# robjermy/CMVS-PMVS

Hardware: AMD Instinct MI355X
Metric: refined patches/sec + NCC evals/sec, 50-view 4K synthetic, 1/2/4/8 GPU (higher is better)
Workload: dtype f32 (f64 optimizer)

## Files before the change

cmvs-pmvs_amd/csrc/pmvs_api.cpp:

```cpp
#include <hip/hip_runtime.h>

#include <algorithm>
#include <climits>
#include <cmath>
#include <cstdarg>
#include <cstdio>
#include <cstdlib>
#include <cstring>
#include <chrono>
#include <condition_variable>
#include <mutex>
#include <string>
#include <vector>

#include "../../include/pmvs_amd.h"
#include "pmvs_features.h"
#include "pmvs_fmt.h"
#include "pmvs_launch.h"

using namespace pmvsdev;

namespace {

thread_local std::string g_err = "";
// ... 1615 lines not shown
  HIPCHK(hipSetDevice(sc->device));
  ExportTemp tmp;
  pmvs_patch* dP = nullptr;
  if (n) {
    EXPCHK(tmp.alloc(&dP, (size_t)n));
    EXPCHK(hipMemcpyAsync(dP, patches, (size_t)n * sizeof(pmvs_patch), hipMemcpyHostToDevice, sc->stream));
  }
  return text_records(sc, dP, n, sz, kind, flags, index2image, out, cap, bytes);
}

pmvs_status pmvs_selftest_format(int32_t device, int32_t precision, const float* in, int32_t n, char* out, int32_t* len) {
  if (!in || !out || !len || n <= 0 || (precision != 6 && precision != 17)) return fail(PMVS_EINVAL, "invalid argument");
  if (device == -1) {
    std::memset(out, 0, (size_t)n * 24);
    for (int i = 0; i < n; ++i) len[i] = pmvsfmt::fmt_g(in[i], precision, out + (size_t)i * 24);
    return PMVS_OK;
  }
  HIPCHK(hipSetDevice(device));
  ExportTemp tmp;
  float* d_in = nullptr;
  char* d_out = nullptr;
  int* d_len = nullptr;
  EXPCHK(tmp.alloc(&d_in, (size_t)n));
  EXPCHK(tmp.alloc(&d_out, (size_t)n * 24));
  EXPCHK(tmp.alloc(&d_len, (size_t)n));
  EXPCHK(hipMemcpy(d_in, in, (size_t)n * sizeof(float), hipMemcpyHostToDevice));
  EXPCHK(hipMemset(d_out, 0, (size_t)n * 24));
  EXPCHK(launch_format_selftest(precision, d_in, n, d_out, d_len, nullptr));
  EXPCHK(hipMemcpy(out, d_out, (size_t)n * 24, hipMemcpyDeviceToHost));
  EXPCHK(hipMemcpy(len, d_len, (size_t)n * sizeof(int), hipMemcpyDeviceToHost));
  return PMVS_OK;
}

pmvs_status pmvs_scene_set_shard(pmvs_scene* sc, int32_t rank, int32_t world, pmvs_allgather_fn fn, void* ctx) {
  if (!sc || world < 1 || rank < 0 || rank >= world || (world > 1 && !fn)) return fail(PMVS_EINVAL, "invalid shard");
  sc->shard_rank = rank;
  sc->shard_world = world;
  sc->shard_fn = fn;
  sc->shard_ctx = ctx;
  sc->shard_rccl = nullptr;
  return PMVS_OK;
}

pmvs_status pmvs_scene_set_cluster(pmvs_scene* sc, int32_t rank, int32_t world, const int32_t* image_ids,
                                   pmvs_allgather_fn fn, void* ctx) {
  if (!sc || world < 1 || rank < 0 || rank >= world || (world > 1 && (!fn || !image_ids)))
    return fail(PMVS_EINVAL, "invalid cluster");
  sc->cl_world = 1;
  sc->cl_fn = nullptr;
  sc->cl_rccl = nullptr;
  if (world == 1) return PMVS_OK;
  const int num = sc->ds.num, tnum = sc->ds.tnum;
  pmvs_status bad = PMVS_OK;
  int maxid = -1;
  std::vector<int> id2idx;
  if (tnum > PMVS_MAX_TARGETS) bad = fail(PMVS_EUNSUPPORTED, "cluster: more than %d target images", PMVS_MAX_TARGETS);
  for (int i = 0; i < num && !bad; ++i) {
    if (image_ids[i] < 0) bad = fail(PMVS_EINVAL, "image_ids[%d] = %d", i, image_ids[i]);
    maxid = std::max(maxid, image_ids[i]);
  }
  if (!bad && maxid > (1 << 26)) bad = fail(PMVS_EUNSUPPORTED, "image number %d", maxid);
  if (!bad) {
    id2idx.assign((size_t)maxid + 1, -1);
    for (int i = 0; i < num && !bad; ++i) {
      if (id2idx[image_ids[i]] >= 0) bad = fail(PMVS_EINVAL, "image number %d appears twice", image_ids[i]);
      id2idx[image_ids[i]] = i;
// ... 105 lines not shown
```

cmvs-pmvs_amd/csrc/pmvs_filter.hip:

```cpp
#include <hip/hip_runtime.h>
#include <hipcub/hipcub.hpp>

#include <algorithm>
#include <chrono>
#include <cmath>
#include <cstdio>
#include <cstddef>
#include <cstdlib>
#include <cstring>
#include <functional>
#include <mutex>
#include <unordered_map>
#include <vector>

#include "pmvs_device.h"
#include "pmvs_launch.h"
#include "pmvs_layout.h"
#include "pmvs_queue.h"

namespace pmvsdev {

#ifndef PMVS_NB_CAP
#define PMVS_NB_CAP 1024
#endif
// ... 2515 lines not shown
  FCHK(memset_big(B.cellcnt, 0, (c.ncells + 1) * sizeof(int), c.st));
  if (e > 0) {
    hipLaunchKernelGGL(cell_hist_kernel, dim3(nblk(e)), dim3(256), 0, c.st, B.keys2, e, B.cellcnt);
    hipLaunchKernelGGL(items_kernel, dim3(nblk(e)), dim3(256), 0, c.st, B.keys2, e, items);
  }
  FCHK(cub_run(B.temp, [&](void* t, size_t& tb) {
    return hipcub::DeviceScan::ExclusiveSum(t, tb, B.cellcnt.p, csr_off, (int)(c.ncells + 1), c.st);
  }));
  return hipGetLastError();
}

__global__ void flag_order_kernel(const int* __restrict__ v, const int* __restrict__ order, int na, int* __restrict__ f) {
  const int i = blockIdx.x * blockDim.x + threadIdx.x;
  if (i < na) f[i] = v[order[i]] != 0;
}
__global__ void scatter_order_kernel(const int* __restrict__ f, const int* __restrict__ off, const int* __restrict__ order,
                                     int na, int* __restrict__ out) {
  const int i = blockIdx.x * blockDim.x + threadIdx.x;
  if (i < na && f[i]) out[off[i]] = order[i];
}

__global__ void pack_bits_kernel(const int* __restrict__ f, int n, unsigned* __restrict__ bits) {
  const int w = blockIdx.x * blockDim.x + threadIdx.x;
  if (w * 32 >= n) return;
  unsigned v = 0u;
  for (int b = 0; b < 32 && w * 32 + b < n; ++b) v |= (f[w * 32 + b] != 0 ? 1u : 0u) << b;
  bits[w] = v;
}
__global__ void unpack_bits_kernel(const unsigned* __restrict__ bits, int n, int* __restrict__ f) {
  const int k = blockIdx.x * blockDim.x + threadIdx.x;
  if (k < n) f[k] = (bits[k >> 5] >> (k & 31)) & 1u;
}

static int lab_jump() {
  static const int v = getenv("PMVS_LAB_JUMP") ? std::max(1, atoi(getenv("PMVS_LAB_JUMP"))) : 1;
  return v;
}
__global__ void lab_init_kernel(int* __restrict__ lab, int* __restrict__ active, int na) {
  const int i = blockIdx.x * blockDim.x + threadIdx.x;
  if (i < na) {
    lab[i] = i;
    active[i] = 1;
  }
}
__global__ void lab_relax_kernel(const int* __restrict__ eoff, const int* __restrict__ edges, int na, int* lab,
                                 int* active, int all, int* changed, int jump) {
  const int i = blockIdx.x * blockDim.x + threadIdx.x;
  if (i >= na) return;
  if (!all && !jump && active[i] == 0) return;
  const int l0 = lab[i], l1 = lab[l0];
  const bool jumped = l1 < l0 && atomicMin(&lab[i], l1) > l1;
  if (jumped) atomicOr(changed, 1);
  if (!all && !jumped && active[i] == 0) return;
  if (atomicExch(&active[i], 0) == 0 && !all && !jumped) return;
  const int li = atomicAdd(&lab[i], 0);
  bool any = false;
  for (int e = eoff[i]; e < eoff[i + 1]; ++e) {
    const int j = edges[e];
    if (li < lab[j] && atomicMin(&lab[j], li) > li) {
      atomicOr(&active[j], 1);
      any = true;
    }
  }
  if (any) atomicOr(changed, 1);
}
__global__ void lab_count_kernel(const int* __restrict__ lab, int na, int* __restrict__ csize) {
  const int i = blockIdx.x * blockDim.x + threadIdx.x;
  const int l = (i < na) ? lab[i] : -1;
  const int l0 = __shfl(l, 0, 64);
  const unsigned long long same = __ballot(i < na && l == l0);
  if (i < na && l != l0) atomicAdd(&csize[l], 1);
  if ((threadIdx.x & 63) == 0 && same) atomicAdd(&csize[l0], (int)__popcll(same));
}
__global__ void lab_flags_kernel(const int* __restrict__ lab, const int* __restrict__ csize, const int* __restrict__ order,
                                 int na, int threshold, int* __restrict__ flags) {
  const int i = blockIdx.x * blockDim.x + threadIdx.x;
  if (i < na && csize[lab[i]] < threshold) flags[order[i]] = 1;
}

static hipError_t collect(Ctx& c) {
  FilterBuffers& B = c.B;
  FCHK(hipMemsetAsync(B.counters, 0, 8 * sizeof(int), c.st));
  hipLaunchKernelGGL(first_cell_kernel, dim3(std::min(nblk((long long)c.n * kLG), 2048u)), dim3(256), 0, c.st, c.s, c.P, c.n,
                     B.preg, B.tgoff, B.keys,
                     B.counters);
  FCHK(cub_run(B.temp, [&](void* t, size_t& tb) {
    return hipcub::DeviceRadixSort::SortKeys(t, tb, B.keys.p, B.keys2.p, c.n, 32, 32 + cell_bits(c.ncells), c.st);
  }));
  FCHK(read_int(B.counters, &c.nalive, c.st));
  FCHK(hipMemsetAsync(B.rank, 0xff, c.n * sizeof(int), c.st));
  if (c.nalive > 0)
    hipLaunchKernelGGL(rank_kernel, dim3(nblk(c.nalive)), dim3(256), 0, c.st, B.keys2, c.nalive, B.order, B.rank);
  hipLaunchKernelGGL(hot_kernel, dim3(nblk(c.n)), dim3(256), 0, c.st, c.s, c.P, c.n, B.hot);
  return hipGetLastError();
}

static hipError_t set_dm_vgrids(Ctx& c, int additive) {
// ... 230 lines not shown
    }
    fprintf(stderr, "[filter] neighbours: max unique %d, overflowed %d of %d; first: %d %d %d\n", mx, ov, c.nalive,
            cnts[ord[0]], c.nalive > 1 ? cnts[ord[1]] : 0, c.nalive > 2 ? cnts[ord[2]] : 0);
  }
  FCHK(read_int(B.counters + 3, overflow, st));
  if (part) {
    long long ovf = 0;
    FCHK(merge_flags(*overflow, &ovf));
    *overflow = (int)ovf;
    if (inject && inj_where == 'g') return hipErrorOutOfMemory;
  }
  {
    int errs[2] = {0, 0};
    FCHK(hipMemcpy(errs, B.counters + 6, 2 * sizeof(int), hipMemcpyDeviceToHost));
    if (errs[0]) {
      fprintf(stderr, "[filter] neighbor kernel bounds violations: %d (first code %d)\n", errs[0], errs[1]);
      return hipErrorIllegalAddress;
    }
  }
  FCHK(apply_flags(c, &counts[2]));
  FCHK(set_dm_vgrids(c, 1));
  if (c.nalive) {
    const int na = c.nalive;
    hipLaunchKernelGGL(group_edges_kernel, dim3(nblk(na)), dim3(256), 0, st, s, c.dev(), 0, B.edge_off, B.cnt, B.edges);
    FCHK(hipMemsetAsync(B.cnt + na, 0, sizeof(int), st));
    FCHK(cub_run(B.temp, [&](void* t, size_t& tb) { return hipcub::DeviceScan::ExclusiveSum(t, tb, B.cnt.p, B.edge_off.p, na + 1, st); }));
    int ne = 0;
    FCHK(read_int(B.edge_off + na, &ne, st));
    if ((size_t)ne > B.edges.cap) FCHK(B.edges.alloc((size_t)ne * 2));
    hipLaunchKernelGGL(group_edges_kernel, dim3(nblk(na)), dim3(256), 0, st, s, c.dev(), 1, B.edge_off, B.cnt, B.edges);
    const int threshold = std::max(20, na / 10000);
    int* lab = B.need;
    int* csize = B.list;
    int* changed = B.counters + 5;
    int* active = B.list;
    hipLaunchKernelGGL(lab_init_kernel, dim3(nblk(na)), dim3(256), 0, st, lab, active, na);
    int sweep = 0;
    for (int it = 0;; ++it) {
      const bool verify = (it % 9) == 8;
      FCHK(hipMemsetAsync(changed, 0, sizeof(int), st));
      for (int r = 0; r < (verify ? 1 : 8); ++r) {
        if (ne)
          hipLaunchKernelGGL(lab_relax_kernel, dim3(nblk(na)), dim3(256), 0, st, B.edge_off, B.edges, na, lab, active,
                             verify ? 1 : 0, changed, (sweep++ % lab_jump()) == 0 ? 1 : 0);
      }
      int ch = 0;
      FCHK(read_int(changed, &ch, st));
      if (verify && !ch) break;
      if (!verify && !ch) it = 9 * (it / 9) + 7;
      if (it > 9 * (na + 1)) return hipErrorIllegalState;
    }
    FCHK(hipMemsetAsync(csize, 0, na * sizeof(int), st));
    hipLaunchKernelGGL(lab_count_kernel, dim3(nblk(na)), dim3(256), 0, st, lab, na, csize);
    FCHK(hipMemsetAsync(B.flags, 0, n * sizeof(int), st));
    hipLaunchKernelGGL(lab_flags_kernel, dim3(nblk(na)), dim3(256), 0, st, lab, csize, B.order, na, threshold, B.flags);
    hipLaunchKernelGGL(flag_rank_kernel, dim3(nblk(na)), dim3(256), 0, st, dP, B.order, na);
    hipLaunchKernelGGL(clear_fixed_kernel, dim3(nblk(n)), dim3(256), 0, st, dP, n, B.flags);
    FCHK(apply_flags(c, &counts[3]));
  }
  dbg(st, "groups");
  FCHK(set_dm_vgrids(c, 1));
  FCHK(build_lists(c, 0));
  FCHK(collect(c));
  hipLaunchKernelGGL(keep_kernel, dim3(nblk(n)), dim3(256), 0, st, n, B.preg, B.rank, keep_dev);
  int lovf = 0;
  FCHK(read_int(B.counters + 8, &lovf, st));
  if (lovf) return hipErrorNotSupported;
  return hipGetLastError();
}

static void nb_prof_dump(const char* what) {
#if defined(NB_PROFILE)
  unsigned long long h[3][8];
  if (hipDeviceSynchronize() != hipSuccess || hipMemcpyFromSymbol(h, HIP_SYMBOL(g_nb_prof), sizeof(h)) != hipSuccess) return;
  fprintf(stderr, "{\"nb_prof\": \"%s\"", what);
  for (int k = 0; k < 3; ++k) {
    fprintf(stderr, ", \"k%d\": [", k);
    for (int i = 0; i < 8; ++i) fprintf(stderr, "%s%llu", i ? ", " : "", h[k][i]);
    fprintf(stderr, "]");
  }
  fprintf(stderr, "}\n");
  std::memset(h, 0, sizeof(h));
  (void)hipMemcpyToSymbol(HIP_SYMBOL(g_nb_prof), h, sizeof(h));
#else
  (void)what;
#endif
}

hipError_t filter_pass(const DScene& s, FilterBuffers& B, pmvs_patch* dP, int n, long long ncells, const long long* h_tgoff,
                       int grid, hipStream_t st, int counts[4], int* overflow, int* keep_dev, const Shard* sh,
                       bool* handled) {
  bool agreed = false;
  hipError_t e = filter_pass_impl(s, B, dP, n, ncells, h_tgoff, grid, st, counts, overflow, keep_dev, sh, agreed);
  nb_prof_dump("filter");
  if (handled) *handled = true;
  if (e != hipSuccess && sh && sh->world > 1 && n > 0 && !agreed) {
    int h[2] = {1, 0};
    std::vector<int> all(2 * (size_t)sh->world, 0);
    (void)sh->exchange(h, sizeof(h), all.data());
  }
  return e;
}


namespace {

static inline float __int_as_float_h(int v) {
  float f;
  std::memcpy(&f, &v, sizeof(f));
  return f;
}

__global__ void count_ok_kernel(const int* __restrict__ ok, int n, int* __restrict__ out) {
  const int i = blockIdx.x * blockDim.x + threadIdx.x;
  const unsigned long long m = __ballot(i < n && ok[i] != 0);
  if ((threadIdx.x & 63) == 0 && m) atomicAdd(out, (int)__popcll(m));
}

__global__ void gather_slots_kernel(const int* __restrict__ slots, int m, const pmvs_candidate* __restrict__ cin,
// ... 1239 lines not shown
```

cmvs-pmvs_amd/csrc/pmvs_launch.h:

```cpp
#pragma once
#include <hip/hip_runtime.h>
#include "pmvs_device.h"
#include "pmvs_devbuf.h"
#include "pmvs_refine_layouts.h"
#include <functional>
#include <memory>
#include <utility>
#include <vector>

namespace pmvsdev {

inline hipError_t memset_big(void* p, int value, size_t bytes, hipStream_t st) {
  constexpr size_t kPiece = size_t(1) << 30;
  char* c = static_cast<char*>(p);
  for (size_t off = 0; off < bytes; off += kPiece) {
    const hipError_t e = hipMemsetAsync(c + off, value, bytes - off < kPiece ? bytes - off : kPiece, st);
    if (e != hipSuccess) return e;
  }
  return hipSuccess;
}
struct PinnedBuf {
  void* p = nullptr;
  size_t cap = 0;
  PinnedBuf() = default;
// ... 77 lines not shown
  const int *image_ids = nullptr, *vimage_ids = nullptr;
};
hipError_t text_offsets(int kind, const TextArrays& in, int n, long long header_bytes, long long* d_off, hipStream_t st);
hipError_t text_write(int kind, const TextArrays& in, int n, const long long* d_off, char* d_out, hipStream_t st);
hipError_t launch_format_selftest(int precision, const float* d_in, int n, char* d_out, int* d_len, hipStream_t st);

struct DepthMapArrays {
  int* patch = nullptr;
  float *depth = nullptr, *normal = nullptr, *ncc = nullptr;
};
hipError_t depth_map_pass(const DScene& s, const pmvs_patch* P, int n, const int* src, const long long* d_off,
                          long long cells, const DepthMapArrays& out, hipStream_t st);

struct alignas(64) PHot {
  float coord[4];
  float normal[4];
  float dscale, ncc, unit0, pad[5];
};
struct FilterBuffers {
  PinnedBuf pin;
  DevBuf<Reg> preg, vreg, safe;
  DevBuf<unsigned long long> keys, keys2, dpkey;
  DevBuf<long long> tgoff;
  DevBuf<int> cnt, off, cellcnt, pg_off, pg_items, vp_off, vp_items, order, rank, flags, need, list, counters, edge_off,
      edges;
  DevBuf<PHot> hot;
  DevBuf<double> scratch;
  DevBuf<char> temp;
  DevBuf<unsigned> rbits;
  DevBuf<float4> coordc;
  DevBuf<unsigned long long> vrows, used;
  DevBuf<float4> normalc;
  DevBuf<int> refpos;
  DevBuf<char> xr;
  DevBuf<float> qf;
  DevBuf<double> qrows;
  DevBuf<int4> qjobs;
  DevBuf<unsigned long long> qctr;
  DevBuf<unsigned long long> qkeys, qkeys2;
  DevBuf<int> qcrows, qoff;
  size_t cap_qrows = 0;
  DevBuf<int> ovf_items;
  DevBuf<double> scratch_big;
  int cap_n = 0, cap_grid = 0;
  long long cap_cells = 0;
  size_t cap_e = 0;
  hipError_t reserve(int n, long long ncells, int tnum, int grid);
  hipError_t ensure_entries(size_t e, int vis);
  void release() { *this = FilterBuffers(); }
};

hipError_t launch_filter_refimage(const DScene& s, pmvs_patch* P, const int* list, int m, int grid, hipStream_t stream,
                                  int* refpos = nullptr, int rank = 0, int world = 1);
hipError_t launch_apply_refpos(const DScene& s, pmvs_patch* P, const int* list, int m, const int* allpos, int world,
                               hipStream_t stream);

constexpr int kMaxWave = 65536;
struct CommitWork;
struct CommitWorkDelete {
  void operator()(CommitWork* w) const;
};
struct H2DStage {
  PinnedBuf pin;
  hipEvent_t done = nullptr;
  bool pending = false;
  H2DStage() = default;
// ... 27 lines not shown
  DevBuf<float> qkey;
  DevBuf<int> qrank, qrank2;
  DevBuf<int> qkeep, qpos;
  DevBuf<int> sflag, spos, slot2;
  DevBuf<char> qitems;
  DevBuf<char> qsort_tmp;
  DevBuf<char> xsd, xrd;
  DevBuf<int> cidx;
  DevBuf<int> crec, acc;
  DevBuf<int2> dupd;
  size_t pool_host = 0;
  std::vector<int> gw, gh;
  void release() { *this = ExpandBuffers(); }
};
using RefineFn = std::function<hipError_t(const pmvs_candidate* d_in, int n, pmvs_refined* d_out)>;
using ExchangeFn = std::function<int(const void* send, size_t bytes, void* recv)>;
using ExchangeDevFn = std::function<int(const void* dsend, size_t bytes, void* drecv, hipStream_t st)>;
struct Shard {
  int rank = 0, world = 1;
  ExchangeFn exchange;
  ExchangeDevFn exchange_dev;
};
hipError_t filter_pass(const DScene& s, FilterBuffers& B, pmvs_patch* dP, int n, long long ncells, const long long* h_tgoff,
                       int grid, hipStream_t st, int counts[4], int* overflow, int* keep_dev, const Shard* sh = nullptr,
                       bool* handled = nullptr);
hipError_t expand_pass(const DScene& s, FilterBuffers& B, ExpandBuffers& X, pmvs_patch*& dP, size_t& dP_cap, int n0,
                       const int* d_alive, int cap, long long ncells, const long long* h_tgoff, int wave, int cthr,
                       int flags, int grid, hipStream_t st, const RefineFn& refine, const Shard& sh, long long stats[8],
                       int* n_out, int min_cands = 0);
using CompactDst = std::function<hipError_t(int, pmvs_patch**)>;
hipError_t compact_model(FilterBuffers& B, const pmvs_patch* src, int n, const int* keep, const CompactDst& dst_for,
                         int* nkept, hipStream_t st);
hipError_t fill_int(int* a, int n, int v, hipStream_t st);
void d2h_stage_release(hipStream_t st);

struct ClusterMaps {
  const unsigned char* shared_t;
  const int* ids;
  const int* id2idx;
  int maxid;
};
struct ClusterBuffers {
  DevBuf<BRec> send, recv;
  DevBuf<pmvs_patch> ins;
  DevBuf<int> flags, pos, cnts;
  DevBuf<char> temp;
};
hipError_t drop_foreign(FilterBuffers& B, const pmvs_patch* src, int n, const CompactDst& dst_for, int* n_out,
                        hipStream_t st);
hipError_t cluster_exchange(const DScene& s, ClusterBuffers& CB, const ClusterMaps& cm, const pmvs_patch* src, int n,
                            pmvs_patch*& dst, size_t& dst_cap, int* n_out, const Shard& sh, hipStream_t st,
                            long long xstats[3], bool& agreed);
hipError_t lls_selftest(const float* A, const float* b, const int* off, int nsys, int total, float* x);

struct SeedInput {
  const pmvs_point* points;
  const int* npts;
  const int* vis_off;
  const int* vis;
  int sequence;
  float angle0;
  std::vector<const uint8_t*> mask_level;
  int batch, per_cell;
  int lookahead;
  int spec_near;
};
// ... 9 lines not shown
```

cmvs-pmvs_amd/pmvs_amd.py:

```python
from __future__ import annotations

import ctypes as C
import os
from dataclasses import dataclass, field
from typing import List, Optional, Sequence

import numpy as np

HERE = os.path.dirname(os.path.abspath(__file__))
LIB_PATH = os.environ.get("PMVS_AMD_LIB", os.path.join(HERE, "libpmvs_amd.so"))

MAX_IMAGES = 128
MAX_TAU = 16

ACCEPTED, FAIL_PRE, FAIL_POST, FAIL_OVERFLOW = 0, 1, 2, 3
FIX_FOREIGN = 2

CANDIDATE_DTYPE = np.dtype(
    [("coord", "<f4", 4), ("normal", "<f4", 4), ("dscale", "<f4"), ("num_images", "<i4"),
     ("images", "<i4", MAX_IMAGES)], align=True)
REFINED_DTYPE = np.dtype(
    [("status", "<i4"), ("refine_code", "<i4"), ("evals", "<i4"), ("num_images", "<i4"),
     ("coord", "<f4", 4), ("normal", "<f4", 4), ("ncc", "<f4"), ("dscale", "<f4"), ("ascale", "<f4"),
     ("tmp", "<f4"), ("timages", "<i4"), ("reserved", "<i4"), ("images", "<i4", MAX_IMAGES),
# ... 97 lines not shown
        return d


class Options(C.Structure):
    _fields_ = [(k, C.c_int32) for k in ("level", "csize", "wsize", "min_image_num", "cpu", "use_bound",
                                          "use_vis_data", "sequence", "tflag", "oflag")] + \
               [(k, C.c_float) for k in ("threshold", "set_edge", "max_angle", "quad")] + \
               [(k, C.c_int32) for k in ("num_timages", "num_oimages", "num_bindexes")] + \
               [(k, C.POINTER(C.c_int32)) for k in ("timages", "oimages", "bindexes", "visdata2_offsets",
                                                      "visdata2")]


class SynthParams(C.Structure):
    _fields_ = [("num_views", C.c_int32), ("num_targets", C.c_int32), ("width", C.c_int32),
                ("height", C.c_int32), ("supersample", C.c_int32), ("level", C.c_int32),
                ("seed", C.c_uint64), ("ring_radius", C.c_double), ("height_offset", C.c_double),
                ("focal_scale", C.c_double), ("arc_step_deg", C.c_double), ("gain_sigma", C.c_double),
                ("bias_sigma", C.c_double), ("noise_sigma", C.c_double), ("lowtex", C.c_double),
                ("occluder_radius", C.c_double), ("render_first", C.c_int32), ("render_count", C.c_int32)]


HARD = dict(gain_sigma=0.15, bias_sigma=0.04, noise_sigma=0.08, lowtex=0.5, occluder_radius=0.3)


EXPORTS = ["pmvs_last_error", "pmvs_device_count", "pmvs_scene_create", "pmvs_scene_destroy",
           "pmvs_set_thresholds", "pmvs_scene_get_level", "pmvs_grab_tex", "pmvs_incc_eval",
           "pmvs_refine_batch", "pmvs_refine_batch_device", "pmvs_scene_sync", "pmvs_synth_ring",
           "pmvs_synth_candidates", "pmvs_selftest_math", "pmvs_selftest_bobyqa", "pmvs_camera_load",
           "pmvs_ppm_load", "pmvs_options_load", "pmvs_options_free", "pmvs_write_patches", "pmvs_write_pset",
           "pmvs_write_ply", "pmvs_patch_colors", "pmvs_filter_run",
           "pmvs_expand_run", "pmvs_expand_fetch", "pmvs_run_loop", "pmvs_loop_fetch", "pmvs_loop_hash",
           "pmvs_loop_export_sizes", "pmvs_loop_export", "pmvs_export_patches_sizes", "pmvs_export_patches",
           "pmvs_depth_map_layout", "pmvs_loop_depth_maps", "pmvs_depth_maps_patches", "pmvs_write_pfm",
           "pmvs_loop_text", "pmvs_text_patches", "pmvs_selftest_format",
           "pmvs_scene_set_shard", "pmvs_scene_set_shard_rccl", "pmvs_scene_set_cluster",
           "pmvs_scene_set_cluster_rccl", "pmvs_rccl_unique_id",
           "pmvs_rccl_create", "pmvs_rccl_destroy", "pmvs_rccl_allgather", "pmvs_rccl_allgather_device",
           "pmvs_tcp_create", "pmvs_tcp_allgather", "pmvs_tcp_destroy", "pmvs_thread_exchange_create",
           "pmvs_thread_exchange_ctx", "pmvs_thread_allgather", "pmvs_thread_exchange_destroy", "pmvs_detect_features",
           "pmvs_seed_run", "pmvs_seed_fetch", "pmvs_selftest_lls", "pmvs_image_load", "pmvs_pnm_mask_load", "pmvs_set_edge"]

ALLGATHER_FN = C.CFUNCTYPE(C.c_int, C.c_void_p, C.c_void_p, C.c_int64, C.c_void_p)

_lib = None


def load_library(path: str = LIB_PATH) -> C.CDLL:
    global _lib
    if _lib is not None:
        return _lib
    if not os.path.exists(path):
        raise RuntimeError(f"{path} not built: run `make -C cmvs-pmvs_amd` (no CPU fallback exists)")
    lib = C.CDLL(path)
    lib.pmvs_last_error.restype = C.c_char_p
    lib.pmvs_device_count.restype = C.c_int32
    lib.pmvs_scene_create.argtypes = [C.POINTER(SceneDesc), C.c_int32, C.POINTER(C.c_void_p)]
    lib.pmvs_scene_destroy.argtypes = [C.c_void_p]
    lib.pmvs_scene_destroy.restype = None
    lib.pmvs_set_thresholds.argtypes = [C.c_void_p, C.c_float, C.c_float, C.c_int32]
    lib.pmvs_scene_get_level.argtypes = [C.c_void_p, C.c_int32, C.c_int32, C.c_void_p,
                                         C.POINTER(C.c_int32), C.POINTER(C.c_int32)]
    lib.pmvs_grab_tex.argtypes = [C.c_void_p, C.c_void_p, C.c_int32, C.c_void_p, C.c_void_p]
    lib.pmvs_detect_features.argtypes = [C.c_void_p, C.c_int32, C.c_int32, C.c_void_p, C.c_int32,
                                         C.POINTER(C.c_int32)]
    lib.pmvs_seed_run.argtypes = [C.c_void_p, C.c_void_p, C.c_void_p, C.c_int32, C.c_void_p, C.c_int32,
                                  C.POINTER(C.c_int32), C.POINTER(SeedStats)]
    lib.pmvs_seed_fetch.argtypes = [C.c_void_p, C.c_void_p, C.c_int32]
# ... 12 lines not shown
    lib.pmvs_image_load.argtypes = [C.c_char_p, C.POINTER(C.c_int32), C.POINTER(C.c_int32), C.c_void_p]
    lib.pmvs_pnm_mask_load.argtypes = [C.c_char_p, C.POINTER(C.c_int32), C.POINTER(C.c_int32), C.c_void_p]
    lib.pmvs_set_edge.argtypes = [C.c_void_p, C.c_int32, C.c_int32, C.c_float, C.c_void_p]
    lib.pmvs_ppm_load.argtypes = [C.c_char_p, C.POINTER(C.c_int32), C.POINTER(C.c_int32), C.c_void_p]
    lib.pmvs_options_load.argtypes = [C.c_char_p, C.c_char_p, C.POINTER(C.POINTER(Options))]
    lib.pmvs_options_free.argtypes = [C.POINTER(Options)]
    lib.pmvs_options_free.restype = None
    lib.pmvs_write_patches.argtypes = [C.c_char_p, C.c_int32] + [C.c_void_p] * 5
    lib.pmvs_write_pset.argtypes = [C.c_char_p, C.c_int32, C.c_void_p]
    lib.pmvs_write_ply.argtypes = [C.c_char_p, C.c_int32, C.c_void_p, C.c_void_p]
    lib.pmvs_patch_colors.argtypes = [C.c_void_p, C.c_int32] + [C.c_void_p] * 4
    lib.pmvs_filter_run.argtypes = [C.c_void_p, C.c_void_p, C.c_int32, C.c_void_p, C.POINTER(FilterStats)]
    lib.pmvs_expand_run.argtypes = [C.c_void_p, C.c_void_p, C.c_void_p, C.c_int32, C.c_int32, C.c_int32, C.c_int32, C.c_int32,
                                    C.c_void_p, C.c_void_p, C.c_int32, C.POINTER(C.c_int32), C.POINTER(ExpandStats)]
    lib.pmvs_expand_fetch.argtypes = [C.c_void_p, C.c_void_p, C.c_void_p, C.c_int32]
    lib.pmvs_run_loop.argtypes = [C.c_void_p, C.c_void_p, C.c_int32, C.c_float, C.c_int32, C.c_int32, C.c_int32, C.c_int32,
                                  C.c_int32, C.POINTER(C.c_int32), C.c_void_p]
    lib.pmvs_loop_fetch.argtypes = [C.c_void_p, C.c_void_p, C.c_int32]
    lib.pmvs_loop_hash.argtypes = [C.c_void_p, C.POINTER(C.c_uint64)]
    lib.pmvs_loop_export_sizes.argtypes = [C.c_void_p, C.POINTER(ExportSizes)]
    lib.pmvs_loop_export.argtypes = [C.c_void_p, C.c_int32, C.c_void_p, C.POINTER(ExportBuffers)]
    lib.pmvs_export_patches_sizes.argtypes = [C.c_void_p, C.c_void_p, C.c_int32, C.POINTER(ExportSizes)]
    lib.pmvs_export_patches.argtypes = [C.c_void_p, C.c_void_p, C.c_int32, C.c_int32, C.c_void_p,
                                        C.POINTER(ExportBuffers)]
    lib.pmvs_depth_map_layout.argtypes = [C.c_void_p, C.c_void_p, C.c_void_p]
    lib.pmvs_loop_depth_maps.argtypes = [C.c_void_p, C.c_int32, C.POINTER(DepthMapBuffers)]
    lib.pmvs_depth_maps_patches.argtypes = [C.c_void_p, C.c_void_p, C.c_int32, C.c_int32, C.POINTER(DepthMapBuffers)]
    lib.pmvs_write_pfm.argtypes = [C.c_char_p, C.c_int32, C.c_int32, C.c_void_p]
    lib.pmvs_loop_text.argtypes = [C.c_void_p, C.c_int32, C.c_int32, C.c_void_p, C.c_void_p, C.c_int64,
                                   C.POINTER(C.c_int64)]
    lib.pmvs_text_patches.argtypes = [C.c_void_p, C.c_void_p, C.c_int32, C.c_int32, C.c_int32, C.c_void_p, C.c_void_p,
                                      C.c_int64, C.POINTER(C.c_int64)]
    lib.pmvs_selftest_format.argtypes = [C.c_int32, C.c_int32, C.c_void_p, C.c_int32, C.c_void_p, C.c_void_p]
    lib.pmvs_scene_set_shard.argtypes = [C.c_void_p, C.c_int32, C.c_int32, C.c_void_p, C.c_void_p]
    lib.pmvs_scene_set_cluster.argtypes = [C.c_void_p, C.c_int32, C.c_int32, C.c_void_p, C.c_void_p, C.c_void_p]
    lib.pmvs_scene_set_cluster_rccl.argtypes = [C.c_void_p, C.c_int32, C.c_int32, C.c_void_p, C.c_void_p]
    lib.pmvs_rccl_unique_id.argtypes = [C.c_void_p]
    lib.pmvs_rccl_create.argtypes = [C.c_int32, C.c_int32, C.c_int32, C.c_void_p, C.POINTER(C.c_void_p)]
    lib.pmvs_rccl_destroy.argtypes = [C.c_void_p]
    lib.pmvs_rccl_destroy.restype = None
    lib.pmvs_rccl_allgather.argtypes = [C.c_void_p, C.c_void_p, C.c_int64, C.c_void_p]
    lib.pmvs_rccl_allgather.restype = C.c_int
    lib.pmvs_scene_set_shard_rccl.argtypes = [C.c_void_p, C.c_int32, C.c_int32, C.c_void_p]
    lib.pmvs_tcp_create.argtypes = [C.c_int32, C.c_int32, C.c_char_p, C.c_int32, C.c_int32, C.POINTER(C.c_void_p)]
    lib.pmvs_tcp_allgather.argtypes = [C.c_void_p, C.c_void_p, C.c_int64, C.c_void_p]
    lib.pmvs_tcp_destroy.argtypes = [C.c_void_p]
    lib.pmvs_tcp_destroy.restype = None
    lib.pmvs_thread_exchange_create.argtypes = [C.c_int32]
    lib.pmvs_thread_exchange_create.restype = C.c_void_p
    lib.pmvs_thread_exchange_ctx.argtypes = [C.c_void_p, C.c_int32]
    lib.pmvs_thread_exchange_ctx.restype = C.c_void_p
    lib.pmvs_thread_allgather.argtypes = [C.c_void_p, C.c_void_p, C.c_int64, C.c_void_p]
    lib.pmvs_thread_exchange_destroy.argtypes = [C.c_void_p]
    lib.pmvs_thread_exchange_destroy.restype = None
    for fn in EXPORTS:
        getattr(lib, fn).restype = getattr(lib, fn).restype or C.c_int
    lib.pmvs_last_error.restype = C.c_char_p
    lib.pmvs_device_count.restype = C.c_int32
    lib.pmvs_scene_destroy.restype = None
    lib.pmvs_options_free.restype = None
    lib.pmvs_thread_exchange_create.restype = C.c_void_p
    lib.pmvs_thread_exchange_ctx.restype = C.c_void_p
    lib.pmvs_thread_exchange_destroy.restype = None
    lib.pmvs_tcp_destroy.restype = None
    _lib = lib
    return lib
# ... 389 lines not shown

def points_flat(points):
    parts = []
    for pv in points:
        if isinstance(pv, np.ndarray) and pv.dtype == POINT_DTYPE:
            parts.append(pv)
            continue
        a = np.asarray(pv, np.float32).reshape(-1, 4)
        r = np.zeros(len(a), POINT_DTYPE)
        r["x"], r["y"], r["response"], r["type"] = a[:, 0], a[:, 1], a[:, 2], a[:, 3].astype(np.int32)
        parts.append(r)
    npts = np.array([len(p) for p in parts], np.int32)
    flat = np.concatenate(parts) if parts and npts.sum() else np.zeros(1, POINT_DTYPE)
    return np.ascontiguousarray(flat), npts


def selftest_math(op: int, x: np.ndarray, device: int = 0) -> np.ndarray:
    x = np.ascontiguousarray(x, np.float64)
    out = np.zeros_like(x)
    _check(load_library().pmvs_selftest_math(device, op, _ptr(x), _ptr(out), len(x)))
    return out


def selftest_format(precision: int, x: np.ndarray, device: int = 0):
    x = np.ascontiguousarray(x, np.float32).reshape(-1)
    out = np.zeros((len(x), 24), np.uint8)
    ln = np.zeros(len(x), np.int32)
    if len(x):
        _check(load_library().pmvs_selftest_format(device, precision, _ptr(x), len(x), _ptr(out), _ptr(ln)))
    raw = out.tobytes()
    return [raw[24 * i:24 * i + int(k)] for i, k in enumerate(ln)]


def selftest_lls(systems, device: int = 0) -> np.ndarray:
    A = np.ascontiguousarray(np.concatenate([np.asarray(a, np.float32).reshape(-1, 5) for a, _ in systems]))
    b = np.ascontiguousarray(np.concatenate([np.asarray(v, np.float32).reshape(-1) for _, v in systems]))
    off = np.zeros(len(systems) + 1, np.int32)
    off[1:] = np.cumsum([len(v) for _, v in systems])
    x = np.zeros((len(systems), 5), np.float32)
    _check(load_library().pmvs_selftest_lls(device, _ptr(A), _ptr(b), _ptr(off), len(systems), _ptr(x)))
    return x


def selftest_bobyqa(kind: int, x0: np.ndarray, mode: int = 0, maxeval: int = 1000, device: int = 0):
    x0 = np.ascontiguousarray(x0, np.float64).reshape(-1, 3)
    out = np.zeros((len(x0), 6), np.float64)
    ms = C.c_double()
    _check(load_library().pmvs_selftest_bobyqa(device, mode, kind, _ptr(x0), len(x0), maxeval, _ptr(out), C.byref(ms)))
    return out, ms.value


def camera_load(path: str) -> np.ndarray:
    out = np.zeros(12, np.float32)
    _check(load_library().pmvs_camera_load(path.encode(), _ptr(out)))
    return out.reshape(3, 4)


def ppm_load(path: str) -> np.ndarray:
    lib = load_library()
    w, h = C.c_int32(), C.c_int32()
    _check(lib.pmvs_ppm_load(path.encode(), C.byref(w), C.byref(h), None))
    img = np.zeros((h.value, w.value, 3), np.uint8)
    _check(lib.pmvs_ppm_load(path.encode(), C.byref(w), C.byref(h), _ptr(img)))
    return img


# ... 237 lines not shown
```

include/pmvs_amd.h:

```cpp
#ifndef PMVS_AMD_H
#define PMVS_AMD_H

#include <stdint.h>

#ifdef __cplusplus
extern "C" {
#endif

#define PMVS_MAX_IMAGES 128
#define PMVS_MAX_TARGETS 256
#define PMVS_MAX_TAU 16
#define PMVS_MAX_LEVEL 4
#define PMVS_MAX_NEIGHBOURS 16384

typedef enum pmvs_status {
  PMVS_OK = 0,
  PMVS_EINVAL = 1,
  PMVS_EDEVICE = 2,
  PMVS_ENOMEM = 3,
  PMVS_EUNSUPPORTED = 4
} pmvs_status;

typedef enum pmvs_candidate_status {
  PMVS_ACCEPTED = 0,
// ... 196 lines not shown
  int64_t* vimage_off;
  int32_t* vimage_ids;
  int32_t* source;
} pmvs_export_buffers;

pmvs_status pmvs_loop_export_sizes(pmvs_scene* scene, pmvs_export_sizes* sizes);
pmvs_status pmvs_loop_export(pmvs_scene* scene, int32_t flags, const int32_t* index2image,
                             const pmvs_export_buffers* buffers);
pmvs_status pmvs_export_patches_sizes(pmvs_scene* scene, const pmvs_patch* patches, int32_t n, pmvs_export_sizes* sizes);
pmvs_status pmvs_export_patches(pmvs_scene* scene, const pmvs_patch* patches, int32_t n, int32_t flags,
                                const int32_t* index2image, const pmvs_export_buffers* buffers);

typedef struct pmvs_depthmap_buffers {
  int32_t* patch;
  float*   depth;
  float*   normal;
  float*   ncc;
} pmvs_depthmap_buffers;

pmvs_status pmvs_depth_map_layout(pmvs_scene* scene, int32_t* dims, int64_t* offsets);
pmvs_status pmvs_loop_depth_maps(pmvs_scene* scene, int32_t flags, const pmvs_depthmap_buffers* buffers);
pmvs_status pmvs_depth_maps_patches(pmvs_scene* scene, const pmvs_patch* patches, int32_t n, int32_t flags,
                                    const pmvs_depthmap_buffers* buffers);

#define PMVS_TEXT_PLY 0
#define PMVS_TEXT_PATCH 1
#define PMVS_TEXT_PSET 2
pmvs_status pmvs_loop_text(pmvs_scene* scene, int32_t kind, int32_t flags, const int32_t* index2image,
                           char* out, int64_t cap, int64_t* bytes);
pmvs_status pmvs_text_patches(pmvs_scene* scene, const pmvs_patch* patches, int32_t n, int32_t kind, int32_t flags,
                              const int32_t* index2image, char* out, int64_t cap, int64_t* bytes);
pmvs_status pmvs_selftest_format(int32_t device, int32_t precision, const float* in, int32_t n,
                                 char* out , int32_t* len );

typedef struct pmvs_seed_stats {
  int64_t trial, pass, fail0, fail1;
  int64_t refined;
  int64_t rounds;
  int64_t candidates;
  int64_t reserved;
  double wall_ms, gen_ms, refine_ms;
} pmvs_seed_stats;
pmvs_status pmvs_seed_run(pmvs_scene* scene, const pmvs_point* points, const int32_t* num_points, int32_t batch,
                          pmvs_patch* out, int32_t cap, int32_t* n_out, pmvs_seed_stats* stats);
pmvs_status pmvs_seed_fetch(pmvs_scene* scene, pmvs_patch* out, int32_t n);

typedef int (*pmvs_allgather_fn)(void* ctx, const void* send, int64_t bytes, void* recv);
pmvs_status pmvs_scene_set_shard(pmvs_scene* scene, int32_t rank, int32_t world, pmvs_allgather_fn fn, void* ctx);

typedef struct pmvs_rccl pmvs_rccl;
pmvs_status pmvs_rccl_unique_id(uint8_t* id128);
pmvs_status pmvs_rccl_create(int32_t device, int32_t rank, int32_t world, const uint8_t* id128, pmvs_rccl** out);
void pmvs_rccl_destroy(pmvs_rccl* comm);
int pmvs_rccl_allgather(void* comm, const void* send, int64_t bytes, void* recv);
int pmvs_rccl_allgather_device(void* comm, const void* dsend, int64_t bytes, void* drecv, void* hip_stream);
pmvs_status pmvs_scene_set_shard_rccl(pmvs_scene* scene, int32_t rank, int32_t world, pmvs_rccl* comm);

pmvs_status pmvs_scene_set_cluster(pmvs_scene* scene, int32_t rank, int32_t world, const int32_t* image_ids,
                                   pmvs_allgather_fn fn, void* ctx);
pmvs_status pmvs_scene_set_cluster_rccl(pmvs_scene* scene, int32_t rank, int32_t world, const int32_t* image_ids,
                                        pmvs_rccl* comm);

typedef struct pmvs_tcp pmvs_tcp;
pmvs_status pmvs_tcp_create(int32_t rank, int32_t world, const char* addr, int32_t port, int32_t timeout_ms,
                            pmvs_tcp** out);
int pmvs_tcp_allgather(void* ctx, const void* send, int64_t bytes, void* recv);
// ... 65 lines not shown
```

Before: 967,900.

## Replace label propagation with union-find hooking plus residual supernode sweeps

```diff
diff --git a/cmvs-pmvs_amd/csrc/pmvs_api.cpp b/cmvs-pmvs_amd/csrc/pmvs_api.cpp
--- a/cmvs-pmvs_amd/csrc/pmvs_api.cpp
+++ b/cmvs-pmvs_amd/csrc/pmvs_api.cpp
@@ -1671,6 +1671,20 @@
   return PMVS_OK;
 }
 
+pmvs_status pmvs_selftest_labels(int32_t device, int32_t n, const int32_t* edge_off, const int32_t* edges, int32_t* lab_out,
+                                 int32_t* stats_out) {
+  if (n <= 0 || !edge_off || !lab_out || !stats_out || edge_off[0] != 0) return fail(PMVS_EINVAL, "invalid argument");
+  for (int i = 0; i < n; ++i)
+    if (edge_off[i + 1] < edge_off[i]) return fail(PMVS_EINVAL, "edge_off decreases at %d", i);
+  if (edge_off[n] > 0 && !edges) return fail(PMVS_EINVAL, "invalid argument");
+  for (int e = 0; e < edge_off[n]; ++e)
+    if (edges[e] < 0 || edges[e] >= n) return fail(PMVS_EINVAL, "edge %d leaves the graph", e);
+  HIPCHK(hipSetDevice(device));
+  const hipError_t e = labels_selftest(edge_off, edges, n, lab_out, stats_out);
+  if (e != hipSuccess) return fail(PMVS_EDEVICE, "labels selftest: %s", hipGetErrorString(e));
+  return PMVS_OK;
+}
+
 pmvs_status pmvs_scene_set_shard(pmvs_scene* sc, int32_t rank, int32_t world, pmvs_allgather_fn fn, void* ctx) {
   if (!sc || world < 1 || rank < 0 || rank >= world || (world > 1 && !fn)) return fail(PMVS_EINVAL, "invalid shard");
   sc->shard_rank = rank;
diff --git a/cmvs-pmvs_amd/csrc/pmvs_filter.hip b/cmvs-pmvs_amd/csrc/pmvs_filter.hip
--- a/cmvs-pmvs_amd/csrc/pmvs_filter.hip
+++ b/cmvs-pmvs_amd/csrc/pmvs_filter.hip
@@ -2571,37 +2571,124 @@
   if (k < n) f[k] = (bits[k >> 5] >> (k & 31)) & 1u;
 }
 
-static int lab_jump() {
-  static const int v = getenv("PMVS_LAB_JUMP") ? std::max(1, atoi(getenv("PMVS_LAB_JUMP"))) : 1;
-  return v;
-}
-__global__ void lab_init_kernel(int* __restrict__ lab, int* __restrict__ active, int na) {
+__global__ void lab_init_kernel(int* __restrict__ parent, int na) {
   const int i = blockIdx.x * blockDim.x + threadIdx.x;
-  if (i < na) {
-    lab[i] = i;
-    active[i] = 1;
-  }
-}
-__global__ void lab_relax_kernel(const int* __restrict__ eoff, const int* __restrict__ edges, int na, int* lab,
-                                 int* active, int all, int* changed, int jump) {
+  if (i < na) parent[i] = i;
+}
+__device__ __forceinline__ int lab_find(int* parent, int x) {
+  int p = parent[x];
+  while (p != x) {
+    const int g = parent[p];
+    if (g != p) atomicMin(&parent[x], g);
+    x = p;
+    p = g;
+  }
+  return x;
+}
+__global__ void lab_hook_kernel(const int* __restrict__ eoff, const int* __restrict__ edges, int na, int* parent) {
   const int i = blockIdx.x * blockDim.x + threadIdx.x;
   if (i >= na) return;
-  if (!all && !jump && active[i] == 0) return;
-  const int l0 = lab[i], l1 = lab[l0];
-  const bool jumped = l1 < l0 && atomicMin(&lab[i], l1) > l1;
-  if (jumped) atomicOr(changed, 1);
-  if (!all && !jumped && active[i] == 0) return;
-  if (atomicExch(&active[i], 0) == 0 && !all && !jumped) return;
-  const int li = atomicAdd(&lab[i], 0);
-  bool any = false;
+  int ri = i;
   for (int e = eoff[i]; e < eoff[i + 1]; ++e) {
     const int j = edges[e];
-    if (li < lab[j] && atomicMin(&lab[j], li) > li) {
-      atomicOr(&active[j], 1);
-      any = true;
-    }
+    if (j <= i) continue;
+    ri = lab_find(parent, ri);
+    int rj = lab_find(parent, j);
+    if (ri == rj) continue;
+    bool mutual = false;
+    for (int f = eoff[j]; f < eoff[j + 1] && !mutual; ++f) mutual = edges[f] == i;
+    if (!mutual) continue;
+    while (ri != rj) {
+      const int hi = max(ri, rj), lo = min(ri, rj);
+      const int old = atomicCAS(&parent[hi], hi, lo);
+      if (old == hi) {
+        ri = rj = lo;
+        break;
+      }
+      ri = lab_find(parent, old);
+      rj = lab_find(parent, lo);
+    }
+  }
+}
+__global__ void lab_flatten_kernel(const int* __restrict__ parent, int na, int* __restrict__ root, int* __restrict__ nsuper) {
+  const int i = blockIdx.x * blockDim.x + threadIdx.x;
+  int x = i;
+  if (i < na) {
+    for (int p = parent[x]; p != x; p = parent[x]) x = p;
+    root[i] = x;
+  }
+  const unsigned long long roots = __ballot(i < na && x == i);
+  if ((threadIdx.x & 63) == 0 && roots) atomicAdd(nsuper, (int)__popcll(roots));
+}
+__global__ void lab_cross_kernel(const int* __restrict__ eoff, const int* __restrict__ edges, const int* __restrict__ root,
+                                 int na, int* __restrict__ cross) {
+  const int i = blockIdx.x * blockDim.x + threadIdx.x;
+  if (i >= na) return;
+  const int ri = root[i];
+  int f = 0;
+  for (int e = eoff[i]; e < eoff[i + 1] && !f; ++e) f = root[edges[e]] != ri;
+  cross[i] = f;
+}
+__global__ void lab_residual_kernel(const int* __restrict__ cross, const int* __restrict__ off, int na, int* __restrict__ rlist) {
+  const int i = blockIdx.x * blockDim.x + threadIdx.x;
+  if (i < na && cross[i]) rlist[off[i]] = i;
+}
+__global__ void lab_sweep_kernel(const int* __restrict__ eoff, const int* __restrict__ edges, const int* __restrict__ root,
+                                 const int* __restrict__ rlist, int nres, int* slab, int* changed) {
+  const int t = blockIdx.x * blockDim.x + threadIdx.x;
+  if (t >= nres) return;
+  const int i = rlist[t], ri = root[i];
+  int li = slab[ri];
+  bool any = false;
+  const int g = slab[li];
+  if (g < li) {
+    any = atomicMin(&slab[ri], g) > g;
+    li = g;
+  }
+  for (int e = eoff[i]; e < eoff[i + 1]; ++e) {
+    const int rj = root[edges[e]];
+    if (rj != ri && li < slab[rj] && atomicMin(&slab[rj], li) > li) any = true;
   }
   if (any) atomicOr(changed, 1);
+}
+__global__ void lab_assign_kernel(const int* __restrict__ slab, int na, int* __restrict__ root) {
+  const int i = blockIdx.x * blockDim.x + threadIdx.x;
+  if (i < na) root[i] = slab[root[i]];
+}
+struct LabelWork {
+  int *parent, *lab, *cross, *off, *rlist, *ctr;
+};
+static hipError_t label_stage(const int* eoff, const int* edges, int na, const LabelWork& W, DevBuf<char>& temp,
+                              hipStream_t st, int* stats) {
+  const dim3 grid(nblk(na)), blk(256);
+  int* const changed = W.ctr;
+  int* const nsuper = W.ctr + 1;
+  FCHK(hipMemsetAsync(W.ctr, 0, 2 * sizeof(int), st));
+  hipLaunchKernelGGL(lab_init_kernel, grid, blk, 0, st, W.parent, na);
+  hipLaunchKernelGGL(lab_hook_kernel, grid, blk, 0, st, eoff, edges, na, W.parent);
+  hipLaunchKernelGGL(lab_flatten_kernel, grid, blk, 0, st, W.parent, na, W.lab, nsuper);
+  hipLaunchKernelGGL(lab_cross_kernel, grid, blk, 0, st, eoff, edges, W.lab, na, W.cross);
+  FCHK(hipMemsetAsync(W.cross + na, 0, sizeof(int), st));
+  FCHK(cub_run(temp, [&](void* t, size_t& tb) { return hipcub::DeviceScan::ExclusiveSum(t, tb, W.cross, W.off, na + 1, st); }));
+  int nres = 0, ns = 0, sweeps = 0;
+  FCHK(d2h_sync(st, {{&nres, W.off + na, sizeof(int)}, {&ns, nsuper, sizeof(int)}}));
+  if (nres) {
+    hipLaunchKernelGGL(lab_residual_kernel, grid, blk, 0, st, W.cross, W.off, na, W.rlist);
+    int* const slab = W.parent;
+    for (int batch = 2;; batch = std::min(2 * batch, 16)) {
+      for (int r = 0; r < batch; ++r)
+        hipLaunchKernelGGL(lab_sweep_kernel, dim3(nblk(nres)), blk, 0, st, eoff, edges, W.lab, W.rlist, nres, slab, changed);
+      sweeps += batch;
+      int ch = 0;
+      FCHK(read_int(changed, &ch, st));
+      if (!ch) break;
+      if (sweeps > 2 * na + 32) return hipErrorIllegalState;
+      FCHK(hipMemsetAsync(changed, 0, sizeof(int), st));
+    }
+    hipLaunchKernelGGL(lab_assign_kernel, grid, blk, 0, st, slab, na, W.lab);
+  }
+  if (stats) stats[0] = ns, stats[1] = nres, stats[2] = sweeps;
+  return hipGetLastError();
 }
 __global__ void lab_count_kernel(const int* __restrict__ lab, int na, int* __restrict__ csize) {
   const int i = blockIdx.x * blockDim.x + threadIdx.x;
@@ -2898,24 +2985,9 @@
     const int threshold = std::max(20, na / 10000);
     int* lab = B.need;
     int* csize = B.list;
-    int* changed = B.counters + 5;
-    int* active = B.list;
-    hipLaunchKernelGGL(lab_init_kernel, dim3(nblk(na)), dim3(256), 0, st, lab, active, na);
-    int sweep = 0;
-    for (int it = 0;; ++it) {
-      const bool verify = (it % 9) == 8;
-      FCHK(hipMemsetAsync(changed, 0, sizeof(int), st));
-      for (int r = 0; r < (verify ? 1 : 8); ++r) {
-        if (ne)
-          hipLaunchKernelGGL(lab_relax_kernel, dim3(nblk(na)), dim3(256), 0, st, B.edge_off, B.edges, na, lab, active,
-                             verify ? 1 : 0, changed, (sweep++ % lab_jump()) == 0 ? 1 : 0);
-      }
-      int ch = 0;
-      FCHK(read_int(changed, &ch, st));
-      if (verify && !ch) break;
-      if (!verify && !ch) it = 9 * (it / 9) + 7;
-      if (it > 9 * (na + 1)) return hipErrorIllegalState;
-    }
+    FCHK(B.lparent.grow_headroom((size_t)na));
+    FCHK(label_stage(B.edge_off, B.edges, na, LabelWork{B.lparent, lab, B.cnt, B.off, B.list, B.counters + 12}, B.temp, st,
+                     nullptr));
     FCHK(hipMemsetAsync(csize, 0, na * sizeof(int), st));
     hipLaunchKernelGGL(lab_count_kernel, dim3(nblk(na)), dim3(256), 0, st, lab, na, csize);
     FCHK(hipMemsetAsync(B.flags, 0, n * sizeof(int), st));
@@ -2951,6 +3023,20 @@
 #else
   (void)what;
 #endif
+}
+
+hipError_t labels_selftest(const int* h_eoff, const int* h_edges, int n, int* h_lab, int stats[3]) {
+  const int ne = h_eoff[n];
+  DevBuf<int> eoff, edges, parent, lab, cross, off, rlist, ctr;
+  DevBuf<char> temp;
+  FCHK(eoff.alloc((size_t)n + 1)); FCHK(edges.alloc((size_t)ne)); FCHK(parent.alloc((size_t)n)); FCHK(lab.alloc((size_t)n));
+  FCHK(cross.alloc((size_t)n + 1)); FCHK(off.alloc((size_t)n + 1)); FCHK(rlist.alloc((size_t)n)); FCHK(ctr.alloc(2));
+  FCHK(hipMemcpy(eoff, h_eoff, ((size_t)n + 1) * sizeof(int), hipMemcpyHostToDevice));
+  if (ne) FCHK(hipMemcpy(edges, h_edges, (size_t)ne * sizeof(int), hipMemcpyHostToDevice));
+  const hipError_t e = label_stage(eoff, edges, n, LabelWork{parent, lab, cross, off, rlist, ctr}, temp, nullptr, stats);
+  d2h_stage_release(nullptr);
+  FCHK(e);
+  return hipMemcpy(h_lab, lab, (size_t)n * sizeof(int), hipMemcpyDeviceToHost);
 }
 
 hipError_t filter_pass(const DScene& s, FilterBuffers& B, pmvs_patch* dP, int n, long long ncells, const long long* h_tgoff,
diff --git a/cmvs-pmvs_amd/csrc/pmvs_launch.h b/cmvs-pmvs_amd/csrc/pmvs_launch.h
--- a/cmvs-pmvs_amd/csrc/pmvs_launch.h
+++ b/cmvs-pmvs_amd/csrc/pmvs_launch.h
@@ -133,6 +133,7 @@
   DevBuf<unsigned long long> vrows, used;
   DevBuf<float4> normalc;
   DevBuf<int> refpos;
+  DevBuf<int> lparent;
   DevBuf<char> xr;
   DevBuf<float> qf;
   DevBuf<double> qrows;
@@ -226,6 +227,7 @@
 hipError_t compact_model(FilterBuffers& B, const pmvs_patch* src, int n, const int* keep, const CompactDst& dst_for,
                          int* nkept, hipStream_t st);
 hipError_t fill_int(int* a, int n, int v, hipStream_t st);
+hipError_t labels_selftest(const int* h_eoff, const int* h_edges, int n, int* h_lab, int stats[3]);
 void d2h_stage_release(hipStream_t st);
 
 struct ClusterMaps {
diff --git a/cmvs-pmvs_amd/pmvs_amd.py b/cmvs-pmvs_amd/pmvs_amd.py
--- a/cmvs-pmvs_amd/pmvs_amd.py
+++ b/cmvs-pmvs_amd/pmvs_amd.py
@@ -153,7 +153,7 @@
            "pmvs_expand_run", "pmvs_expand_fetch", "pmvs_run_loop", "pmvs_loop_fetch", "pmvs_loop_hash",
            "pmvs_loop_export_sizes", "pmvs_loop_export", "pmvs_export_patches_sizes", "pmvs_export_patches",
            "pmvs_depth_map_layout", "pmvs_loop_depth_maps", "pmvs_depth_maps_patches", "pmvs_write_pfm",
-           "pmvs_loop_text", "pmvs_text_patches", "pmvs_selftest_format",
+           "pmvs_loop_text", "pmvs_text_patches", "pmvs_selftest_format", "pmvs_selftest_labels",
            "pmvs_scene_set_shard", "pmvs_scene_set_shard_rccl", "pmvs_scene_set_cluster",
            "pmvs_scene_set_cluster_rccl", "pmvs_rccl_unique_id",
            "pmvs_rccl_create", "pmvs_rccl_destroy", "pmvs_rccl_allgather", "pmvs_rccl_allgather_device",
@@ -232,6 +232,7 @@
     lib.pmvs_text_patches.argtypes = [C.c_void_p, C.c_void_p, C.c_int32, C.c_int32, C.c_int32, C.c_void_p, C.c_void_p,
                                       C.c_int64, C.POINTER(C.c_int64)]
     lib.pmvs_selftest_format.argtypes = [C.c_int32, C.c_int32, C.c_void_p, C.c_int32, C.c_void_p, C.c_void_p]
+    lib.pmvs_selftest_labels.argtypes = [C.c_int32, C.c_int32, C.c_void_p, C.c_void_p, C.c_void_p, C.c_void_p]
     lib.pmvs_scene_set_shard.argtypes = [C.c_void_p, C.c_int32, C.c_int32, C.c_void_p, C.c_void_p]
     lib.pmvs_scene_set_cluster.argtypes = [C.c_void_p, C.c_int32, C.c_int32, C.c_void_p, C.c_void_p, C.c_void_p]
     lib.pmvs_scene_set_cluster_rccl.argtypes = [C.c_void_p, C.c_int32, C.c_int32, C.c_void_p, C.c_void_p]
@@ -687,6 +688,17 @@
     return [raw[24 * i:24 * i + int(k)] for i, k in enumerate(ln)]
 
 
+def selftest_labels(edge_off: np.ndarray, edges: np.ndarray, device: int = 0):
+    edge_off = np.ascontiguousarray(edge_off, np.int32).reshape(-1)
+    edges = np.ascontiguousarray(edges, np.int32).reshape(-1)
+    n = len(edge_off) - 1
+    lab = np.zeros(max(n, 0), np.int32)
+    stats = np.zeros(3, np.int32)
+    keep = edges if len(edges) else np.zeros(1, np.int32)
+    _check(load_library().pmvs_selftest_labels(device, n, _ptr(edge_off), _ptr(keep), _ptr(lab), _ptr(stats)))
+    return lab, {"supernodes": int(stats[0]), "residual": int(stats[1]), "sweeps": int(stats[2])}
+
+
 def selftest_lls(systems, device: int = 0) -> np.ndarray:
     A = np.ascontiguousarray(np.concatenate([np.asarray(a, np.float32).reshape(-1, 5) for a, _ in systems]))
     b = np.ascontiguousarray(np.concatenate([np.asarray(v, np.float32).reshape(-1) for _, v in systems]))
diff --git a/include/pmvs_amd.h b/include/pmvs_amd.h
--- a/include/pmvs_amd.h
+++ b/include/pmvs_amd.h
@@ -252,6 +252,8 @@
                               const int32_t* index2image, char* out, int64_t cap, int64_t* bytes);
 pmvs_status pmvs_selftest_format(int32_t device, int32_t precision, const float* in, int32_t n,
                                  char* out , int32_t* len );
+pmvs_status pmvs_selftest_labels(int32_t device, int32_t n, const int32_t* edge_off, const int32_t* edges,
+                                 int32_t* lab_out , int32_t* stats_out );
 
 typedef struct pmvs_seed_stats {
   int64_t trial, pass, fail0, fail1;
```

After: 988,800 (median of 6 runs). +2.2%, better.
